# kalenforn/clip-based-cross-modal-hash

Measured on AMD Instinct MI355X. Metric: Hamming query x gallery pairs/sec (fused mAP@all pass, DCMHT COCO-shaped 64-bit), higher is better.
Workload: dtype u32; 1 GPU; configs[1] DCMHT COCO 64-bit retrieval: Q=5000 queries x R=117218 gallery items per GPU (x1 GPUs, contiguous shards), K=64 bits, C=80 classes, mAP@all; Q=5000, R_per_gpu=117218, K=64, C=80, parallelism=gallery-shard x1, query_blocks=1

## Files before the change

### clip-based-cross-modal-hash_amd/csrc/xmh_scan.hip

```cpp
#include "xmh_common.h"
#include <atomic>
#include <math.h>
#include <mutex>
#include <string.h>
#include <vector>
#include "xmh_scan_bits.h"
#include "xmh_scan_mfma.h"
#include "xmh_scan_kernels.h"

#include <stdlib.h>
#include <type_traits>
#include <unordered_set>

namespace {

constexpr int kSlotBudget64 = 9 * 1024;
constexpr int kSlotBudget32 = 5 * 1024;
constexpr int slots_for(int W, bool tern, int counter_bytes) {
    const int nbmax = (tern ? 64 : 32) * W + 1;
    const int budget = counter_bytes == 8 ? kSlotBudget64 : kSlotBudget32;
    const int cap = W > 8 ? 64 : 8;
    int S = 2;
    while (S < cap && nbmax * (64 / S) * counter_bytes > budget) S *= 2;
    return S;
}
inline int instance_words(int W) { return W <= 1 ? 1 : (W <= 2 ? 2 : (W <= 4 ? 4 : (W <= 8 ? 8 : (W <= 16 ? 16 : (W <= 32 ? 32 : 64))))); }
constexpr bool pair_cache_shape(int W, bool tern) { return !tern && (W == 1 || W == 2 || W == 4 || W == 8); }
template <int W, bool TERN>
constexpr bool kPairCacheShape = pair_cache_shape(W, TERN);
constexpr int cache_slots(int W) { return W <= 2 ? 4 : 8; }
static_assert(slots_for(2, false, 4) == 4 && slots_for(2, false, 8) == 4 && slots_for(4, false, 4) == 8 && slots_for(4, false, 8) == 8 &&
              slots_for(8, false, 4) == 8 && slots_for(8, false, 8) == 8, "33..256 bits: the cache geometry is the uncached kernels' own");
constexpr int waves_for(int W, bool tern) { return (W >= 32 && !tern) ? 8 : 1; }
inline size_t aos_ring_bytes(int W, int LW, bool tern) { return (size_t)64 * (((W * (tern ? 2 : 1) + LW) + 3) / 4 * 4) * 4; }

struct WsLayout {
    size_t chunk_hist, below, tot, dpre, cap, tick, gate, ap_part, pair_cache, total;
};

bool r2_selfcheck_ok();
inline bool mfma_env_on() {
    const char* e = getenv("XMH_SCAN_MFMA");
    return !(e && atoi(e) == 0);
}
struct Overrides {
    int mfma = -1;
    bool masked = false;
    bool describe = false;
};
enum class Family { kValu, kR2, kR2w, kBits, kTBits };
Family pass1_family(int K, bool ternary, const Overrides& ov) {
    if (ov.mfma == 0 || !mfma_env_on()) return Family::kValu;
    if (ternary) return K <= 256 ? Family::kTBits : Family::kValu;
    if (K > 128) return K <= 256 ? Family::kBits : Family::kValu;
    if (ov.mfma < 0 && !r2_selfcheck_ok()) return Family::kValu;
    return K <= 64 ? Family::kR2 : Family::kR2w;
}
inline int tbits_tiles(int K) { return K <= 64 ? 2 : (K <= 128 ? 4 : 8); }
inline int ap_r2_mode() {
    const char* e = getenv("XMH_SCAN_AP_R2");
    return e ? (atoi(e) != 0 ? 1 : 0) : 2;
}
constexpr int kAp2Waves = 4, kAp2Groups = 2;
constexpr int kMfmaWaves = 4;
static_assert(xmh::kScanBitsWaves == kMfmaWaves, "k_scan_hist_b takes the plan's query tiles of 64");
// ... 174 lines not shown
}

int packed_rank_bits(int K, int64_t R) {
    const char* e = getenv("XMH_SCAN_PACK32");
    if (e && e[0] == '0') return 0;
    if (!(K > 64 || (e && e[0] == 'a'))) return 0;
    const int64_t rank_max = R + 2;
    int rank_bits = 0;
    while ((1ll << rank_bits) < rank_max) ++rank_bits;
    return rank_bits > 24 ? 0 : rank_bits;
}

enum class Mode { kUnsharded, kBaseAll, kTotals, kAllToAll };
struct ScanCall {
    const uint32_t *qbits, *qzero, *qlab, *rbits, *rzero, *rlab;
    int64_t Q, R; int K, C;
    void* ws; size_t ws_bytes;
    bool tern;
};
struct Pass2 {
    Mode mode; int64_t k;
    double* ap_sum; int32_t* cap;
    double* map_out;
    const uint32_t *base_all = nullptr, *base_rel = nullptr, *nrel_total = nullptr;
    const uint32_t* hist_g = nullptr;
    int world = 0, rank = 0;
};
enum class Kern { kHistS, kHistR2, kHistR2w, kHistB, kApS, kApC, kApR2 };
enum Gate : unsigned {
    kBySize = 1,
    kByWrap = 2,
    kByWidth = 4,
};
struct Launch {
    Kern kern = Kern::kHistS;
    int W = 0, LW = 0;
    bool tern = false, cache = false;
    int S = 0, NW = 1;
    int nml = 0;
    int eb = 0; bool half = false;
    bool p32 = false, masked = false;
    unsigned gate = 0;
    bool stand_in = false;
};
struct ScanRoute {
    Launch p1;
    size_t cache_bytes = 0;
    int rank_bits = 0;
    Launch p2[3];
    int n2 = 0;
    bool tables32 = false;
};

std::mutex g_packed_mu;
std::unordered_set<const void*> g_packed_ws;
bool ws_packed(const void* ws) { std::lock_guard<std::mutex> lock(g_packed_mu); return g_packed_ws.count(ws) != 0; }
void ws_set_packed(const void* ws, bool on) {
    std::lock_guard<std::mutex> lock(g_packed_mu);
    if (on) g_packed_ws.insert(ws); else g_packed_ws.erase(ws);
}
bool counts_fit16(int K, int64_t R) {
    double peak = 1.0;
    for (int i = 1; i <= K / 2; ++i) peak *= (double)(K - K / 2 + i) / (double)i;
    peak = ldexp(peak, -K);
    return 2.0 * peak * (double)R <= 65535.0;
}
bool tables_packed(bool apc_alone, Mode mode, int K, int64_t R) { return apc_alone && mode == Mode::kUnsharded && counts_fit16(K, R); }

ScanRoute scan_route(const xmh_scan_plan& p, const ScanCall& c, Mode mode, const Overrides& ov, hipStream_t st) {
    ScanRoute r;
    const int K = c.K, C = c.C; const bool tern = c.tern; const int64_t R = c.R;
    const Family fam = pass1_family(K, tern, ov);
    const int W = ov.describe ? instance_words((K + 31) / 32) : (K + 31) / 32, LW = (C + 31) / 32;
    const bool lane_ok = ov.describe || (!ov.masked && lane_order_ok(st));
    r.cache_bytes = cache_for_workspace(p, K, tern, fam, c.ws_bytes);
    const bool cache = r.cache_bytes != 0;
    const bool mfma = fam != Family::kValu && LW <= 4 && lane_ok;
    Launch& h = r.p1;
    h.W = W; h.LW = LW; h.tern = tern; h.cache = cache; h.nml = LW <= 2 ? 1 : 2;
    if (!mfma) {
        h.cache = cache && pair_cache_shape(W, tern);
        h.S = h.cache ? cache_slots(W) : slots_for(W, tern, 4);
        h.NW = h.S == 64 ? waves_for(W, tern) : 1;
    } else if (fam == Family::kBits || fam == Family::kTBits) {
        h.kern = Kern::kHistB;
        h.S = fam == Family::kTBits ? tbits_tiles(K) : 4;
    } else {
        const R2Geom g = r2_geom(K);
        h.kern = fam == Family::kR2 ? Kern::kHistR2 : Kern::kHistR2w;
        h.NW = g.nw; h.S = g.nq;
    }
    const bool sharded = mode != Mode::kUnsharded;
    const bool masked = !lane_ok;
    const int rank_bits = sharded || masked ? 0 : packed_rank_bits(K, R);
    const bool fits_fb = sharded || R <= kFloatBitsMaxItems;
    const bool apc_on = ap_c_on();
    const bool byte128 = cache && mfma && fam == Family::kR2w;
    const bool tb = cache && mfma && fam == Family::kTBits;
    const bool apc = cache && apc_on && (byte128 || (K <= 64 && rank_bits == 0)) && !tern && !masked && (mode != Mode::kBaseAll || byte128) && fits_fb;
    const bool apr2 = !cache && mfma && fam == Family::kR2 && ap_r2_mode() != 0 && !masked && mode != Mode::kBaseAll && rank_bits == 0 && fits_fb;
    const bool apc16 = cache && apc_on && ((K > 128 && K <= 256 && !tern) || tb) && !masked && !sharded && R <= kFloatBitsMaxItems;
    const unsigned size_gate = sharded && (apc || apr2) ? kBySize : 0u;
    r.rank_bits = byte128 && apc ? 0 : rank_bits;
    auto add = [&](Kern kern, unsigned gate) -> Launch& { Launch& l = r.p2[r.n2++]; l.kern = kern; l.gate = gate; return l; };
    if (apc) {
        Launch& l = add(Kern::kApC, size_gate | (byte128 ? kByWrap : 0u));
        l.eb = 8; l.half = byte128; l.S = byte128 ? 8 : 4;
    }
    if (apr2) {
        Launch& l = add(Kern::kApR2, size_gate);
        l.W = W; l.LW = LW; l.nml = h.nml; l.NW = kAp2Waves; l.S = kAp2Groups;
    }
// ... 63 lines not shown
}

MfmaArgs r2_args(const ScanCall& c, const Launch& l, const xmh_scan_plan& p, int nqt) {
    MfmaArgs a{c.qbits, (int)c.Q, (int)c.R, c.K, l.W, (int)p.chunk, (int)p.nchunk, nqt, (int)p.nbuckets, (int)p.qpad};
    a.rbits = c.rbits; a.rlab = c.rlab; a.qlab = c.qlab; a.LW = l.LW;
    return a;
}

struct Geom { unsigned grid, block; size_t lds; int nqt, nrun; };
Geom launch_geom(const Launch& l, const xmh_scan_plan& p, int64_t Q) {
    const size_t nb = (size_t)p.nbuckets;
    const bool ap = l.kern == Kern::kApS || l.kern == Kern::kApC || l.kern == Kern::kApR2;
    Geom g{0, 64u * (unsigned)l.NW, 0, 0};
    if (l.kern == Kern::kHistS || l.kern == Kern::kApS) {
        g.lds = ((nb * (64 / l.S) * (ap && !l.p32 ? 2 : 1) + 3) & ~(size_t)3) * 4 * l.NW + (ap && l.cache ? 0 : aos_ring_bytes(l.W, l.LW, l.tern));
        g.nqt = (int)p.nqtile * l.S / l.NW;
    } else if (l.kern == Kern::kApC) {
        g.lds = nb * (64 / l.S) * 8; g.nqt = (int)p.nqtile * l.S;
    } else if (l.kern == Kern::kHistB) {
        g.nqt = (int)(p.qpad / (16 * kMfmaWaves));
    } else if (l.kern == Kern::kHistR2 || l.kern == Kern::kHistR2w) {
        g.lds = r2_lds_bytes(l.S, (int)nb); g.nqt = (int)(p.qpad / (l.NW * l.S * 16));
    } else {
        g.lds = (size_t)l.NW * l.S * nb * 16 * (ap ? 8 : 4); g.nqt = (int)(p.qpad / (l.NW * l.S * 16));
    }
    g.nrun = g.nqt;
    if (ap) {
        static const bool all_tiles = xmh_experiment_env("XMH_AP_TILES") && atoi(xmh_experiment_env("XMH_AP_TILES")) == 0;
        if (!all_tiles) g.nrun = (int)xmh::ceil_div(Q, p.qpad / g.nqt);
    }
    g.grid = xmh::scan_grid_blocks(g.nrun, (int)p.nchunk);
    return g;
}

template <typename KernT, typename... Args>
int start(const char* who, const Launch& l, const Geom& g, hipStream_t st, KernT kern, int S, int NW, bool cache, Args... args) {
    if (l.S != S || l.NW != NW || l.cache != cache)
        return xmh::fail(XMH_ENOTSUP, "%s: the route names an instance with S=%d NW=%d cache=%d, the one compiled for W=%d LW=%d has S=%d NW=%d cache=%d", who, l.S,
                         l.NW, (int)l.cache, l.W, l.LW, S, NW, (int)cache);
    if (const int rc = xmh::raise_dynamic_lds(reinterpret_cast<const void*>(kern), g.lds, who)) return rc;
    hipLaunchKernelGGL(kern, dim3(g.grid), dim3(g.block), g.lds, st, args...);
    return XMH_OK;
}

struct ScanCtx {
    const ScanCall& c;
    hipStream_t st;
    xmh_scan_plan p;
    ScanRoute r;
    WsLayout L;
    ScanArgs a;
    uint32_t kcap = 0xffffffffu;
    bool capped = false;
    template <typename T> T* at(size_t off) const { return reinterpret_cast<T*>(static_cast<char*>(c.ws) + off); }
    uint32_t* chunk_hist() const { return at<uint32_t>(L.chunk_hist); }
    uint32_t rel_scale() const { return r.p1.kern != Kern::kHistS ? kRelHi16 : 0u; }
    const uint2* below() const { return at<uint2>(L.below); }
    uint2* tot() const { return at<uint2>(L.tot); }
    uint2* dpre() const { return at<uint2>(L.dpre); }
    uint32_t* cap_ws() const { return at<uint32_t>(L.cap); }
    float* ap_part() const { return at<float>(L.ap_part); }
    ScanArgs args(const Geom& g, bool cached) const { ScanArgs as = a; as.nqt = g.nqt; as.nrun = g.nrun; as.pair_cache = cached ? pair_cache() : nullptr; return as; }
    uint32_t* gate(int word = 0) const { return at<uint32_t>(L.gate) + word; }
    const uint32_t* gate_if(const Launch& l, unsigned g, int word) const { return (l.gate & g) ? gate(word) : nullptr; }
    uint4* pair_cache() const { return r.cache_bytes ? at<uint4>(L.pair_cache) : nullptr; }
};

int plan_call(const char* who, ScanCtx& x, const Overrides& ov) {
    if (const int rc = make_plan(x.c.Q, x.c.R, x.c.K, x.c.tern, &x.p, ov)) return rc;
    return check_common(who, x.c, x.p);
}
void route_call(ScanCtx& x, Mode mode, const Overrides& ov) {
    x.r = scan_route(x.p, x.c, mode, ov, x.st);
    x.a = make_args(x.c, x.p);
    x.L = ws_layout(x.p, x.r.cache_bytes);
}

int valu_hist(const ScanCtx& x) {
    const Launch& h = x.r.p1;
    const Geom g = launch_geom(h, x.p, x.c.Q);
    const ScanArgs as = x.args(g, h.cache);
    auto go = [&](auto kern, int S, int NW, bool cache) {
        xmh::ProfScope prof("scan_hist", x.st);
        return start("xmh_hamming_hist", h, g, x.st, kern, S, NW, cache, as, x.chunk_hist());
    };
    auto launch = [&](auto tern_c) {
        constexpr bool T = decltype(tern_c)::value;
        return dispatch_shape<T>(h.W, h.LW, [&](auto w, auto l) {
            constexpr int WW = decltype(w)::value, LL = decltype(l)::value;
            if constexpr (kPairCacheShape<WW, T>) {
                if (h.cache) return go(k_scan_hist_s<WW, LL, T, cache_slots(WW), 1, true>, cache_slots(WW), 1, true);
            }
            constexpr int S = slots_for(WW, T, 4);
            constexpr int NW = S == 64 ? waves_for(WW, T) : 1;
            return go(k_scan_hist_s<WW, LL, T, S, NW, false>, S, NW, false);
        });
    };
    return h.tern ? launch(std::true_type{}) : launch(std::false_type{});
}

int mfma_hist(const ScanCtx& x) {
    const Launch& h = x.r.p1;
    const xmh_scan_plan& p = x.p;
    const Geom g = launch_geom(h, p, x.c.Q);
    uint32_t* chunk_hist = x.chunk_hist();
    uint4* cache = x.pair_cache();
    if (h.kern == Kern::kHistB) {
        xmh::ScanBitsArgs a{x.c.rbits, x.c.rlab, x.c.qbits, x.c.qlab, (int)x.c.Q, (int)x.c.R, x.c.K, h.W, h.LW, (int)p.chunk, (int)p.nchunk, g.nqt,
                            (int)p.nbuckets, (int)p.qpad};
        a.rzero = x.c.rzero; a.qzero = x.c.qzero;
        return xmh::launch_scan_hist_bits(a, h.S, chunk_hist, cache, x.st);
    }
    hipLaunchKernelGGL(k_scan_touch, dim3(xmh::scan_grid_blocks(kTouchPerChunk, (int)p.nchunk)), dim3(256), 0, x.st, x.c.rbits, x.c.rlab, x.c.R, h.W, h.LW,
                       p.chunk, (int)p.nchunk, x.at<uint32_t>(x.L.tick), (int)((x.L.gate + 256 - x.L.tick) / 4));
    XMH_LAUNCH_CHECK("xmh_hamming_hist control words");
    const MfmaArgs a = r2_args(x.c, h, p, g.nqt);
    xmh::ProfScope prof("scan_hist", x.st);
    auto go = [&](auto kern, int NW, int NQ, bool cached, auto... wrap_word) { return start("xmh_hamming_hist", h, g, x.st, kern, NQ, NW, cached, a, chunk_hist, cache, wrap_word...); };
    if (h.kern == Kern::kHistR2w) {
        uint32_t* ovf = x.gate(kGateWrapped);
        return h.nml == 1 ? (h.cache ? go(k_scan_hist_r2w<1, 4, 2, true>, 4, 2, true, ovf) : go(k_scan_hist_r2w<1, 4, 2, false>, 4, 2, false, ovf))
                          : (h.cache ? go(k_scan_hist_r2w<2, 4, 2, true>, 4, 2, true, ovf) : go(k_scan_hist_r2w<2, 4, 2, false>, 4, 2, false, ovf));
    }
    return h.nml == 1 ? (h.cache ? go(k_scan_hist_r2<1, 4, 4, true>, 4, 4, true) : go(k_scan_hist_r2<1, 4, 4, false>, 4, 4, false))
                      : (h.cache ? go(k_scan_hist_r2<2, 4, 4, true>, 4, 4, true) : go(k_scan_hist_r2<2, 4, 4, false>, 4, 4, false));
}

int hamming_hist_impl(const ScanCall& c, uint32_t* hist_all, uint32_t* hist_rel, xmh_stream_t stream, const Overrides& ov, bool pass2_sharded = false) {
    ScanCtx x{c, xmh::as_stream(stream)};
    if (const int rc = plan_call("xmh_hamming_hist", x, ov)) return rc;
    route_call(x, Mode::kUnsharded, ov);
    const xmh_scan_plan& p = x.p;
    const Kern kern = x.r.p1.kern;
    const bool packed = x.r.tables32 && !pass2_sharded;
    if (kern == Kern::kHistS || kern == Kern::kHistB) XMH_HIP(hipMemsetAsync(x.at<char>(x.L.tick), 0, x.L.gate + 256 - x.L.tick, x.st));
    if (const int rc = kern == Kern::kHistS ? valu_hist(x) : mfma_hist(x)) return rc;
    XMH_LAUNCH_CHECK("xmh_hamming_hist");
    hipLaunchKernelGGL(k_scan_below, dim3((unsigned)p.nqtile, (unsigned)xmh::ceil_div(p.nbuckets, 4)), dim3(256), 0, x.st, x.chunk_hist(), (int)p.qpad,
                       (int)p.nbuckets, (int)p.nchunk, x.rel_scale(), x.at<uint2>(x.L.below), x.tot(), x.at<uint32_t>(x.L.tick), (int)c.Q, x.dpre(),
                       x.cap_ws(), x.gate(), hist_all, hist_rel, packed, x.gate(kGateWide));
    XMH_LAUNCH_CHECK("xmh_hamming_hist below");
    ws_set_packed(c.ws, packed);
    return XMH_OK;
}

}

extern "C" int xmh_scan_plan_make(int64_t Q, int64_t R, int K, int ternary, xmh_scan_plan* plan_host) {
    if (!plan_host) return xmh::fail(XMH_EINVAL, "xmh_scan_plan_make: null plan");
    return make_plan(Q, R, K, ternary, plan_host);
}

extern "C" size_t xmh_scan_pair_cache_bytes(int64_t Q, int64_t R, int K, int ternary) {
    xmh_scan_plan p;
    if (make_plan(Q, R, K, ternary, &p)) return 0;
    return pair_cache_bytes(p, K, ternary != 0, pass1_family(K, ternary != 0, {}));
}

extern "C" size_t xmh_scan_pair_cache_offset(int64_t Q, int64_t R, int K, int ternary) {
    xmh_scan_plan p;
    if (make_plan(Q, R, K, ternary, &p)) return (size_t)-1;
    return ws_layout(p, 0).pair_cache;
}

extern "C" size_t xmh_scan_ws_bytes_nocache(int64_t Q, int64_t R, int K, int ternary) {
    xmh_scan_plan p;
    if (make_plan(Q, R, K, ternary, &p)) return 0;
    return ws_layout(p, 0).total;
}

extern "C" int xmh_scan_describe(int64_t Q, int64_t R, int K, int C, int ternary, char* out, size_t out_bytes) {
    if (!out || out_bytes < 64) return xmh::fail(XMH_EINVAL, "xmh_scan_describe: buffer too small");
    xmh_scan_plan p;
    if (const int rc = make_plan(Q, R, K, ternary, &p)) return rc;
    Overrides ov;
    ov.describe = true;
    const ScanCall c{nullptr, nullptr, nullptr, nullptr, nullptr, nullptr, Q, R, K, C, nullptr, (size_t)p.ws_bytes, ternary != 0};
    const ScanRoute r = scan_route(p, c, Mode::kUnsharded, ov, nullptr);
    char p1[160], p2[200] = "", one[120];
    if (const int rc = describe_launch(r.p1, p1, sizeof(p1))) return rc;
    for (const bool p32 : {true, false})
        for (int i = 0; i < r.n2; ++i) {
            if (r.p2[i].stand_in || r.p2[i].p32 != p32) continue;
            if (const int rc = describe_launch(r.p2[i], one, sizeof(one))) return rc;
            const size_t at = strlen(p2);
            snprintf(p2 + at, sizeof(p2) - at, "%s%s", at ? "|" : "", one);
        }
    if ((size_t)snprintf(out, out_bytes, "pass1=%s;pass2=%s", p1, p2) >= out_bytes) return xmh::fail(XMH_EINVAL, "xmh_scan_describe: buffer too small");
    return XMH_OK;
}

extern "C" size_t xmh_scan_gate_offset(int64_t Q, int64_t R, int K, int ternary) {
    xmh_scan_plan p;
    if (make_plan(Q, R, K, ternary, &p)) return (size_t)-1;
    return ws_layout(p, 0).gate;
// ... 2 lines not shown
extern "C" int xmh_scan_tables_packed(int64_t Q, int64_t R, int K, int C, int ternary, int mode) {
    if (mode < 0 || mode > 3) return xmh::fail(XMH_EINVAL, "xmh_scan_tables_packed: mode=%d", mode);
    xmh_scan_plan p;
    if (const int rc = make_plan(Q, R, K, ternary, &p)) return rc;
    Overrides ov;
    ov.describe = true;
    const ScanCall c{nullptr, nullptr, nullptr, nullptr, nullptr, nullptr, Q, R, K, C, nullptr, (size_t)p.ws_bytes, ternary != 0};
    static const Mode modes[4] = {Mode::kUnsharded, Mode::kBaseAll, Mode::kTotals, Mode::kAllToAll};
    return scan_route(p, c, modes[mode], ov, nullptr).tables32 ? 1 : 0;
}

extern "C" int xmh_hamming_hist(const uint32_t* qbits, const uint32_t* qzero, const uint32_t* qlab,
                                const uint32_t* rbits, const uint32_t* rzero, const uint32_t* rlab, int64_t Q, int64_t R,
                                int K, int C, void* ws, size_t ws_bytes, uint32_t* hist_all, uint32_t* hist_rel,
                                xmh_stream_t stream) {
    XMH_RANGE("xmh_hamming_hist (pass 1)");
    const ScanCall c{qbits, qzero, qlab, rbits, rzero, rlab, Q, R, K, C, ws, ws_bytes, qzero != nullptr};
    return hamming_hist_impl(c, hist_all, hist_rel, stream, {}, hist_all != nullptr || hist_rel != nullptr);
}

extern "C" int xmh_hamming_hist_for(const uint32_t* qbits, const uint32_t* qzero, const uint32_t* qlab,
                                    const uint32_t* rbits, const uint32_t* rzero, const uint32_t* rlab, int64_t Q, int64_t R,
                                    int K, int C, void* ws, size_t ws_bytes, uint32_t* hist_all, uint32_t* hist_rel, int pass2_sharded,
                                    xmh_stream_t stream) {
    XMH_RANGE("xmh_hamming_hist (pass 1)");
    const ScanCall c{qbits, qzero, qlab, rbits, rzero, rlab, Q, R, K, C, ws, ws_bytes, qzero != nullptr};
    return hamming_hist_impl(c, hist_all, hist_rel, stream, {}, pass2_sharded != 0);
}

namespace {
int ap_offsets(const ScanCtx& x, const Pass2& o) {
    const xmh_scan_plan& p = x.p;
    if (o.mode == Mode::kUnsharded) return XMH_OK;
    if (o.mode == Mode::kAllToAll)
        hipLaunchKernelGGL(k_shard_scatter_offsets, dim3((unsigned)xmh::ceil_div(p.qpad, 256), (unsigned)p.nbuckets + 1), dim3(256), 0, x.st,
                           reinterpret_cast<const uint2*>(o.hist_g), (int)p.nbuckets, (int)(p.qpad / o.world), (int)x.c.Q, (int)p.qpad, o.k, x.dpre(), x.cap_ws(),
                           o.cap, x.gate(2));
    else if (o.mode == Mode::kTotals)
        hipLaunchKernelGGL(k_shard_offsets_dpre, dim3((unsigned)p.nqtile), dim3(256), 0, x.st, reinterpret_cast<const uint2*>(o.hist_g), o.world, o.rank,
                           (int)x.c.Q, (int)p.qpad, (int)p.nbuckets, o.k, x.dpre(), x.cap_ws(), o.cap, x.gate(2));
    else
        hipLaunchKernelGGL(k_scan_dpre, dim3((unsigned)p.nqtile), dim3(256), 0, x.st, (const uint2*)x.tot(), (int)x.c.Q, (int)p.qpad, (int)p.nbuckets, o.base_all,
                           o.base_rel, o.nrel_total, o.k, x.dpre(), x.cap_ws(), o.cap, (uint32_t*)nullptr, (uint32_t*)nullptr, (uint32_t*)nullptr, x.gate(2));
    XMH_LAUNCH_CHECK(o.mode == Mode::kAllToAll ? "xmh_hamming_map_sharded_offsets scatter" : (o.mode == Mode::kTotals ? "xmh_hamming_map_sharded offsets" : "xmh_hamming_ap dpre"));
    return XMH_OK;
}

int ap_launch_c(const ScanCtx& x, const Launch& l) {
    const Geom g = launch_geom(l, x.p, x.c.Q);
    const ScanArgs as = x.args(g, true);
    const uint32_t* wide = x.r.tables32 ? x.gate(kGateWide) : nullptr;
    xmh::ProfScope prof("scan_ap", x.st);
    auto go = [&](auto kc, int S) {
        return start("xmh_hamming_ap", l, g, x.st, kc, S, 1, l.cache, as, x.below(), (const uint2*)x.dpre(), (const uint32_t*)x.cap_ws(), x.ap_part(),
                     x.gate_if(l, kBySize, 2), x.kcap, x.gate_if(l, kByWrap, kGateWrapped), x.gate_if(l, kByWidth, 0), l.gate & kByWidth ? x.r.rank_bits : 0, wide,
                     (const uint32_t*)x.chunk_hist(), x.rel_scale());
    };
    if (l.eb == 16) return x.capped ? go(k_scan_ap_c<true, 16>, 8) : go(k_scan_ap_c<false, 16>, 8);
    if (l.half) return x.capped ? go(k_scan_ap_c<true, 8, true>, 8) : go(k_scan_ap_c<false, 8, true>, 8);
    return x.capped ? go(k_scan_ap_c<true, 8>, 4) : go(k_scan_ap_c<false, 8>, 4);
}

int ap_launch_r2(const ScanCtx& x, const Launch& l) {
    const Geom g = launch_geom(l, x.p, x.c.Q);
    const MfmaArgs ma = r2_args(x.c, l, x.p, g.nrun);
    xmh::ProfScope prof("scan_ap", x.st);
    auto go = [&](auto kern) {
        return start("xmh_hamming_ap", l, g, x.st, kern, kAp2Groups, kAp2Waves, l.cache, ma, x.below(), (const uint2*)x.dpre(), (const uint32_t*)x.cap_ws(), x.ap_part(),
                     x.gate_if(l, kBySize, 2), x.kcap);
    };
    return l.nml == 1 ? (x.capped ? go(k_scan_ap_r2<1, kAp2Waves, kAp2Groups, true>) : go(k_scan_ap_r2<1, kAp2Waves, kAp2Groups, false>))
                      : (x.capped ? go(k_scan_ap_r2<2, kAp2Waves, kAp2Groups, true>) : go(k_scan_ap_r2<2, kAp2Waves, kAp2Groups, false>));
}

int ap_launch_s(const ScanCtx& x, const Launch& l) {
    const Geom g = launch_geom(l, x.p, x.c.Q);
    const ScanArgs as = x.args(g, l.cache);
    auto go = [&](auto kern, int S, int NW, bool cache, const uint32_t* run_if) {
        xmh::ProfScope prof(l.p32 ? "scan_ap32" : "scan_ap", x.st);
        return start("xmh_hamming_ap", l, g, x.st, kern, S, NW, cache, as, x.below(), (const uint2*)x.dpre(), (const uint32_t*)x.cap_ws(), x.ap_part(),
                     (const uint32_t*)x.gate(), x.r.rank_bits, x.kcap, x.gate_if(l, kBySize, 2), run_if);
    };
    auto by_shape = [&](auto tern_c, auto cap_c, auto p32_c, auto masked_c) {
        constexpr bool T = decltype(tern_c)::value, CP = decltype(cap_c)::value, P32 = decltype(p32_c)::value, MK = decltype(masked_c)::value;
        return dispatch_shape<T>(l.W, l.LW, [&](auto w, auto lw) {
            constexpr int WW = decltype(w)::value, LL = decltype(lw)::value;
            if constexpr (P32 && MK) return xmh::fail(XMH_ENOTSUP, "xmh_hamming_ap: the masked fallback runs 64-bit counters only");
            else {
                if constexpr (kPairCacheShape<WW, T> && !MK) {
                    if (l.cache)
                        return go(k_scan_ap_s<WW, 1, T, CP, cache_slots(WW), P32, MK, 1, true>, cache_slots(WW), 1, true, nullptr);
                }
                (void)CP;
                constexpr int S = slots_for(WW, T, P32 ? 4 : 8);
                constexpr int NW = S == 64 ? waves_for(WW, T) : 1;
                return go(k_scan_ap_s<WW, LL, T, true, S, P32, MK, NW, false>, S, NW, false, x.gate_if(l, kByWrap, kGateWrapped));
            }
        });
    };
    using T1 = std::true_type; using T0 = std::false_type;
    auto by_mask = [&](auto t, auto c, auto w) { return l.masked ? by_shape(t, c, w, T1{}) : by_shape(t, c, w, T0{}); };
    auto by_width = [&](auto t, auto c) { return l.p32 ? by_mask(t, c, T1{}) : by_mask(t, c, T0{}); };
    auto by_cap = [&](auto t) { return x.capped ? by_width(t, T1{}) : by_width(t, T0{}); };
    return l.tern ? by_cap(T1{}) : by_cap(T0{});
}

int ap_reduce(const ScanCtx& x, const Pass2& o) {
    const int64_t Q = x.c.Q;
    const unsigned nred = (unsigned)xmh::ceil_div(Q, 64);
// ... 15 lines not shown

static std::atomic<int> g_verify{0};
constexpr int XMH_EVERIFY_CODE = -74;

int hamming_ap_impl(const ScanCall& c, const Pass2& o, xmh_stream_t stream, const Overrides& ov);

int verify_against_masked(const ScanCall& c, const Pass2& o, xmh_stream_t stream) {
    hipStream_t st = xmh::as_stream(stream);
    const int64_t Q = c.Q;
    std::vector<double> a1((size_t)Q), a0((size_t)Q);
    std::vector<int32_t> c1((size_t)Q), c0((size_t)Q);
    XMH_HIP(hipMemcpyAsync(a1.data(), o.ap_sum, (size_t)Q * 8, hipMemcpyDeviceToHost, st));
    XMH_HIP(hipMemcpyAsync(c1.data(), o.cap, (size_t)Q * 4, hipMemcpyDeviceToHost, st));
    XMH_HIP(hipStreamSynchronize(st));
    Overrides ov;
    ov.mfma = 0;
    ov.masked = true;
    xmh_scan_plan p;
    if (const int rc = make_plan(Q, c.R, c.K, c.tern, &p, ov)) return rc;
    const size_t small = ws_layout(p, 0).total;
    DevBuf ws2, ap2, cap2;
    if (!ws2.alloc(small) || !ap2.alloc((size_t)Q * 8) || !cap2.alloc((size_t)Q * 4))
        return xmh::fail(XMH_ENOMEM, "xmh_scan_verify: no room for the second evaluation (%zu bytes)", small);
    ScanCall again = c; again.ws = ws2.p; again.ws_bytes = small;
    const Pass2 o2{Mode::kUnsharded, o.k, ap2.as<double>(), cap2.as<int32_t>(), nullptr};
    if (const int rc = hamming_hist_impl(again, nullptr, nullptr, stream, ov)) return rc;
    if (const int rc = hamming_ap_impl(again, o2, stream, ov)) return rc;
    XMH_HIP(hipMemcpyAsync(a0.data(), ap2.p, (size_t)Q * 8, hipMemcpyDeviceToHost, st));
    XMH_HIP(hipMemcpyAsync(c0.data(), cap2.p, (size_t)Q * 4, hipMemcpyDeviceToHost, st));
    XMH_HIP(hipStreamSynchronize(st));
    if (const char* fe = getenv("XMH_SCAN_VERIFY_FAULT")) {
        const int64_t at = atoll(fe) % Q;
        a1[(size_t)at] *= 1.0 + 1e-3;
    }
    int64_t bad = -1, nbad = 0;
    for (int64_t i = 0; i < Q; ++i) {
        const bool same = c1[(size_t)i] == c0[(size_t)i] && fabs(a1[(size_t)i] - a0[(size_t)i]) <= 4e-6 * fabs(a0[(size_t)i]) + 1e-9;
        if (!same) { if (bad < 0) bad = i; ++nbad; }
    }
    if (nbad)
        return xmh::fail(XMH_EVERIFY_CODE, "xmh_scan_verify: %lld of %lld queries differ between the lane-order kernels and the masked re-derivation "
                         "(first: query %lld, AP sum %.9g vs %.9g, divisor %d vs %d)", (long long)nbad, (long long)Q, (long long)bad, a1[(size_t)bad], a0[(size_t)bad],
                         c1[(size_t)bad], c0[(size_t)bad]);
    return XMH_OK;
}

int hamming_ap_impl(const ScanCall& c, const Pass2& o, xmh_stream_t stream, const Overrides& ov) {
    ScanCtx x{c, xmh::as_stream(stream)};
    if (const int rc = plan_call("xmh_hamming_ap", x, ov)) return rc;
    if (!o.ap_sum || !o.cap) return xmh::fail(XMH_EINVAL, "xmh_hamming_ap: null output");
    const int ext = (o.base_all != nullptr) + (o.base_rel != nullptr) + (o.nrel_total != nullptr);
    if (ext != 0 && ext != 3) return xmh::fail(XMH_EINVAL, "xmh_hamming_ap: base_all, base_rel and nrel_total go together");
    route_call(x, o.mode, ov);
    const bool have_packed = ws_packed(c.ws);
    if (x.r.tables32 && !have_packed) x.r.tables32 = false;
    x.kcap = o.k > 0 && o.k < (int64_t)0xffffffffll ? (uint32_t)o.k : 0xffffffffu;
    x.capped = o.k > 0;
    if (!x.r.tables32 && have_packed) {
        const xmh_scan_plan& p = x.p;
        hipLaunchKernelGGL(k_scan_below, dim3((unsigned)p.nqtile, (unsigned)xmh::ceil_div(p.nbuckets, 4)), dim3(256), 0, x.st, x.chunk_hist(), (int)p.qpad,
                           (int)p.nbuckets, (int)p.nchunk, x.rel_scale(), x.at<uint2>(x.L.below), x.tot(), (uint32_t*)nullptr, (int)x.c.Q, (uint2*)nullptr,
                           (uint32_t*)nullptr, (uint32_t*)nullptr, (uint32_t*)nullptr, (uint32_t*)nullptr, false, (uint32_t*)nullptr);
        XMH_LAUNCH_CHECK("xmh_hamming_ap below");
        ws_set_packed(c.ws, false);
    }
    if (const int rc = ap_offsets(x, o)) return rc;
    for (int i = 0; i < x.r.n2; ++i) {
        const Launch& l = x.r.p2[i];
        if (const int rc = l.kern == Kern::kApC ? ap_launch_c(x, l) : (l.kern == Kern::kApR2 ? ap_launch_r2(x, l) : ap_launch_s(x, l))) return rc;
        XMH_LAUNCH_CHECK("xmh_hamming_ap");
    }
    if (const int rc = ap_reduce(x, o)) return rc;
    if (g_verify.load(std::memory_order_relaxed) && !ov.masked && o.mode == Mode::kUnsharded) return verify_against_masked(c, o, stream);
    return XMH_OK;
}

bool selfcheck_eval(const ScanCall& c, int force, std::vector<uint32_t>& hist, std::vector<double>& ap, std::vector<int32_t>& cap) {
    Overrides ov;
    ov.mfma = force;
    const int64_t Q = c.Q;
    xmh_scan_plan p;
    if (make_plan(Q, c.R, c.K, 0, &p, ov) != XMH_OK) return false;
    const size_t nb = (size_t)p.nbuckets;
    DevBuf ws, dh, dap, dcap;
    if (!ws.alloc(p.ws_bytes) || !dh.alloc(2 * Q * nb * 4) || !dap.alloc(Q * 8) || !dcap.alloc(Q * 4)) return false;
    ScanCall run = c; run.ws = ws.p; run.ws_bytes = p.ws_bytes;
    const Pass2 o{Mode::kUnsharded, 0, dap.as<double>(), dcap.as<int32_t>(), nullptr};
    uint32_t* h = dh.as<uint32_t>();
    if (hamming_hist_impl(run, h, h + Q * nb, nullptr, ov) != XMH_OK) return false;
    if (hamming_ap_impl(run, o, nullptr, ov) != XMH_OK) return false;
    hist.resize(2 * Q * nb); ap.resize(Q); cap.resize(Q);
    if (hipDeviceSynchronize() != hipSuccess) return false;
    return hipMemcpy(hist.data(), dh.p, hist.size() * 4, hipMemcpyDeviceToHost) == hipSuccess && hipMemcpy(ap.data(), dap.p, Q * 8, hipMemcpyDeviceToHost) == hipSuccess &&
           hipMemcpy(cap.data(), dcap.p, Q * 4, hipMemcpyDeviceToHost) == hipSuccess;
}

bool r2_selfcheck_ok() {
    static int state[64];
    static std::mutex mu;
    int dev = 0;
    if (hipGetDevice(&dev) != hipSuccess || dev < 0 || dev >= 64) return true;
    const char* e = getenv("XMH_SCAN_M2_SELFCHECK");
    if (e && atoi(e) == 0) return true;
    std::lock_guard<std::mutex> lock(mu);
    if (state[dev]) return state[dev] == 1;
    state[dev] = 1;
    const int64_t Q = 272, R = 9000;
    bool same = true, ran = true;
    {
        const void* const r2_kernels[] = {reinterpret_cast<const void*>(k_scan_hist_r2<1, 4, 4, true>), reinterpret_cast<const void*>(k_scan_hist_r2<1, 4, 4, false>),
                                          reinterpret_cast<const void*>(k_scan_hist_r2<2, 4, 4, true>), reinterpret_cast<const void*>(k_scan_hist_r2<2, 4, 4, false>),
                                          reinterpret_cast<const void*>(k_scan_hist_r2w<1, 4, 2, true>), reinterpret_cast<const void*>(k_scan_hist_r2w<1, 4, 2, false>),
                                          reinterpret_cast<const void*>(k_scan_hist_r2w<2, 4, 2, true>), reinterpret_cast<const void*>(k_scan_hist_r2w<2, 4, 2, false>)};
        for (const void* k : r2_kernels) {
            hipFuncAttributes fa;
            if (hipFuncGetAttributes(&fa, k) != hipSuccess) ran = false;
            else if (fa.sharedSizeBytes != 0) same = false;
// ... 160 lines not shown
```

### clip-based-cross-modal-hash_amd/csrc/xmh_scan_kernels.h

```cpp
#pragma once
#include "xmh_scan_mfma.h"

namespace {
template <int W, int LW, bool TERN>
struct QueryRegs {
    uint32_t b[W];
    uint32_t z[TERN ? W : 1];
    uint32_t l[LW];
    __device__ __forceinline__ void load(const ScanArgs& a, int q) {
        const bool ok = q < a.Q;
#pragma unroll
        for (int w = 0; w < W; ++w) b[w] = ok ? a.qbits[(int64_t)q * W + w] : 0u;
        if (TERN) {
#pragma unroll
            for (int w = 0; w < W; ++w) z[w] = ok ? a.qzero[(int64_t)q * W + w] : 0xffffffffu;
        }
#pragma unroll
        for (int w = 0; w < LW; ++w) l[w] = ok ? a.qlab[(int64_t)q * LW + w] : 0u;
    }
};

template <int W, int LW, bool TERN>
struct Rec {
    uint32_t b[W];
// ... 7 lines not shown
        int acc = 0;
#pragma unroll
        for (int w = 0; w < W; ++w) acc += __popc(qr.b[w] ^ r.b[w]);
        d = acc;
    } else {
        int live_n = 0, diff_n = 0;
#pragma unroll
        for (int w = 0; w < W; ++w) {
            const uint32_t live = ~(qr.z[w] | r.z[w]);
            live_n += __popc(live);
            diff_n += __popc((qr.b[w] ^ r.b[w]) & live);
        }
        d = K - live_n + 2 * diff_n;
    }
    uint32_t hit = qr.l[0] & r.l[0];
#pragma unroll
    for (int w = 1; w < LW; ++w) asm("v_and_or_b32 %0, %1, %2, %0" : "+v"(hit) : "v"(qr.l[w]), "v"(r.l[w]));
    asm("v_min_u32 %0, %1, 1" : "=v"(hit01) : "v"(hit));
}

constexpr int kGateWrapped = 3;
constexpr int kGateWide = 4;
__global__ __launch_bounds__(256) void k_scan_below(const uint32_t* __restrict__ chunk_hist, int qpad, int nb, int nchunk, uint32_t rel_scale,
                                                    uint2* __restrict__ below, uint2* __restrict__ tot, uint32_t* __restrict__ tickets, int Q,
                                                    uint2* __restrict__ dpre, uint32_t* __restrict__ nrel_ws, uint32_t* __restrict__ nrel_max,
                                                    uint32_t* __restrict__ hist_all, uint32_t* __restrict__ hist_rel, bool packed,
                                                    uint32_t* __restrict__ wide) {
    __shared__ uint2 part[4][64];
    __shared__ int last;
    const int lane = threadIdx.x & 63, wq = threadIdx.x >> 6;
    const int d = blockIdx.y * 4 + wq;
    const int q = blockIdx.x * 64 + lane;
    const bool hi16 = rel_scale == kRelHi16;
    if (d < nb && packed) {
        const int64_t cell = (int64_t)d * qpad + q, step = (int64_t)nb * qpad;
        const uint32_t* __restrict__ src = chunk_hist + cell;
        uint32_t* __restrict__ dst = reinterpret_cast<uint32_t*>(below) + cell;
        uint32_t ra = 0, rr = 0;
        for (int c0 = 0; c0 < nchunk; c0 += 16) {
            uint32_t h[16];
#pragma unroll
            for (int j = 0; j < 16; ++j, src += step) h[j] = c0 + j < nchunk ? *src : 0u;
#pragma unroll
            for (int j = 0; j < 16; ++j, dst += step) {
                if (c0 + j < nchunk) {
                    *dst = (ra << 16) | rr;
                    const uint2 n = chunk_counts(h[j], rel_scale);
                    ra += n.x;
                    rr += n.y;
                }
            }
        }
        if (ra > 0xffffu && q < Q) *wide = 1u;
        __hip_atomic_store(reinterpret_cast<unsigned long long*>(tot + (int64_t)d * qpad + q), (unsigned long long)ra | ((unsigned long long)rr << 32),
                           __ATOMIC_RELAXED, __HIP_MEMORY_SCOPE_AGENT);
    } else if (d < nb) {
        uint32_t ra = 0, rr = 0;
        int c = 0;
        for (; c + 4 <= nchunk; c += 4) {
            uint32_t h[4];
#pragma unroll
            for (int j = 0; j < 4; ++j) h[j] = chunk_hist[((int64_t)(c + j) * nb + d) * qpad + q];
#pragma unroll
            for (int j = 0; j < 4; ++j) {
                below[((int64_t)(c + j) * nb + d) * qpad + q] = make_uint2(ra, rr);
                const uint32_t rel = hi16 ? h[j] & 0xffffu : (rel_scale ? h[j] / rel_scale : h[j] >> 16);
                ra += hi16 ? h[j] >> 16 : (rel_scale ? h[j] - rel * rel_scale : h[j] & 0xffffu);
                rr += rel;
            }
        }
        for (; c < nchunk; ++c) {
            const uint32_t h = chunk_hist[((int64_t)c * nb + d) * qpad + q];
            below[((int64_t)c * nb + d) * qpad + q] = make_uint2(ra, rr);
            const uint32_t rel = hi16 ? h & 0xffffu : (rel_scale ? h / rel_scale : h >> 16);
            ra += hi16 ? h >> 16 : (rel_scale ? h - rel * rel_scale : h & 0xffffu);
            rr += rel;
        }
        __hip_atomic_store(reinterpret_cast<unsigned long long*>(tot + (int64_t)d * qpad + q), (unsigned long long)ra | ((unsigned long long)rr << 32),
                           __ATOMIC_RELAXED, __HIP_MEMORY_SCOPE_AGENT);
    }
    if (!tickets) return;
    asm volatile("s_waitcnt vmcnt(0)" ::: "memory");
    __syncthreads();
    if (threadIdx.x == 0) {
        const uint32_t t = __hip_atomic_fetch_add(tickets + blockIdx.x, 1u, __ATOMIC_RELAXED, __HIP_MEMORY_SCOPE_AGENT);
        last = t == gridDim.y - 1;
    }
    __syncthreads();
    if (!last) return;
    auto tot_at = [&](int dd) {
        const unsigned long long v = __hip_atomic_load(reinterpret_cast<const unsigned long long*>(tot + (int64_t)dd * qpad + q), __ATOMIC_RELAXED,
                                                       __HIP_MEMORY_SCOPE_AGENT);
        return make_uint2((uint32_t)v, (uint32_t)(v >> 32));
    };
    const int nbq = (nb + 3) / 4;
    const int d0 = wq * nbq, d1 = (d0 + nbq < nb) ? d0 + nbq : nb;
    uint32_t sa = 0, sr = 0;
    for (int dd = d0; dd < d1; dd += 8) {
        uint2 t[8];
#pragma unroll
        for (int j = 0; j < 8; ++j) t[j] = dd + j < d1 ? tot_at(dd + j) : make_uint2(0u, 0u);
#pragma unroll
        for (int j = 0; j < 8; ++j) { sa += t[j].x; sr += t[j].y; }
    }
    part[wq][lane] = make_uint2(sa, sr);
    __syncthreads();
    uint32_t ra = 0, rr = 0, tr = 0;
#pragma unroll
// ... 841 lines not shown
```

### clip-based-cross-modal-hash_amd/csrc/xmh_scan_mfma.h

```cpp
#pragma once
#include "xmh_common.h"
#include "xmh_scan_map.h"
#include <type_traits>
#include <utility>

namespace {

constexpr int kMaxChunk = 32768;
constexpr uint32_t kF23 = 0x4B000000u;
constexpr int64_t kFloatBitsMaxItems = (1ll << 23) - 3;
constexpr int kMinChunk = 256;
constexpr uint32_t kRelHi16 = 0xffffffffu;
__device__ __forceinline__ uint2 chunk_counts(uint32_t h, uint32_t rel_scale) {
    if (rel_scale == kRelHi16) return make_uint2(h >> 16, h & 0xffffu);
    if (rel_scale == 0u) return make_uint2(h & 0xffffu, h >> 16);
    return make_uint2(h % rel_scale, h / rel_scale);
}

struct ScanArgs {
    const uint32_t* qbits;
    const uint32_t* qzero;
    const uint32_t* qlab;
    const uint32_t* rbits;
    const uint32_t* rzero;
// ... 573 lines not shown
            uint32_t i0, i1, i2, i3;
            consume(i0, i1, i2, i3, A[3]);
            if (CACHE) pack(cw[NQ - 1][3], addr_p, i0, i1, i2, i3);
        }
#ifdef XMH_ABL_NOSTORE
        if (CACHE && a.Q < 0) {
#else
        if (CACHE) {
#endif
#pragma unroll
            for (int h = 0; h < NQ; ++h) {
                uint4* dst = crow[h] + (int64_t)i * 64;
                __builtin_nontemporal_store(cw[h][0], &dst->x);
                __builtin_nontemporal_store(cw[h][1], &dst->y);
                __builtin_nontemporal_store(cw[h][2], &dst->z);
                __builtin_nontemporal_store(cw[h][3], &dst->w);
            }
        }
#pragma unroll
        for (int g = 0; g < 4; ++g)
#pragma unroll
            for (int m = 0; m < NMI; ++m) wcur[g][m] = wnxt[g][m];
    }
    const int npad = nbat * 64 - (int)(hi - lo);
    asm volatile("s_waitcnt lgkmcnt(0)" ::: "memory");
    if (npad > 0 && slot == 0) {
#pragma unroll
        for (int h = 0; h < NQ; ++h) {
            if (!valid[h]) continue;
            const int64_t q = (int64_t)(t16 + h) * 16 + ql;
            int dpad = 0;
            for (int w = 0; w < a.W; ++w) dpad += __popc(a.qbits[q * a.W + w]);
            lds[r2_cell(wave, h, dpad, ql)] -= (uint32_t)npad << 16;
        }
    }
#pragma unroll
    for (int h = 0; h < NQ; ++h) {
        uint32_t* __restrict__ out = chunk_hist + ((int64_t)chunk_id * a.nb) * a.qpad + (t16 + h) * 16;
        for (int e = lane; e < ncell; e += 64) out[(int64_t)(e >> 4) * a.qpad + (e & 15)] = lds[r2_cell(wave, h, e >> 4, e & 15)];
    }
    if (CACHE && dmax >= 65536u) *ovf = 1u;
}
#undef XMH_W_FUSED
#undef XMH_W_MFMA_F4
#undef XMH_W_MFMA
#undef XMH_W_MIN
#undef XMH_W_ADD

template <bool CAPPED, int EB, bool HALF = false>
__global__ __launch_bounds__(64) void k_scan_ap_c(ScanArgs a, const uint2* __restrict__ below, const uint2* __restrict__ dpre,
                                                  const uint32_t* __restrict__ cap_ws, float* __restrict__ ap_part,
                                                  const uint32_t* __restrict__ items_total, uint32_t kcap, const uint32_t* __restrict__ skip_if = nullptr,
                                                  const uint32_t* __restrict__ nrel_max = nullptr, int rank_bits = 0, const uint32_t* __restrict__ wide = nullptr,
                                                  const uint32_t* __restrict__ chunk_hist = nullptr, uint32_t rel_scale = 0) {
    static_assert(!HALF || EB == 8, "the 8 x 8 geometry on one-byte entries");
    constexpr int QW = HALF ? 8 : 128 / EB, LOG_QW = QW == 16 ? 4 : 3, S = 64 / QW, EPW = HALF ? 2 : 32 / EB;
    extern __shared__ __attribute__((aligned(16))) uint32_t lds[];
    int chunk_id, qtile;
    if (!map_block(a, chunk_id, qtile)) return;
    if (items_total && (int64_t)*items_total > kFloatBitsMaxItems) return;
    if (skip_if && *skip_if != 0u) return;
    if (nrel_max && rank_bits > 0 && (uint64_t)(*nrel_max) + 2 < (1ull << (32 - rank_bits))) return;
    const int lane = threadIdx.x & 63;
    const int ql = lane & (QW - 1), slot = lane >> LOG_QW;
    const int q0 = qtile * QW, q = q0 + ql;
    const int ncell = a.nb * QW;
    unsigned long long* cnt = reinterpret_cast<unsigned long long*>(lds);
    {
        const uint2* __restrict__ pb = below + ((int64_t)chunk_id * a.nb) * a.qpad + q0;
        const uint2* __restrict__ pd = dpre + q0;
        auto pack = [](uint2 x, uint2 y) {
            return (unsigned long long)(kF23 + x.x + y.x + 1u) | ((unsigned long long)(kF23 + (0x7fffffu - (x.y + y.y + 1u))) << 32);
        };
        int e = lane;
        if (wide == nullptr) {
            for (; e + 7 * 64 < ncell; e += 8 * 64) {
                uint2 x[8], y[8];
#pragma unroll
                for (int j = 0; j < 8; ++j) {
                    const int ee = e + j * 64;
                    const int64_t at = (int64_t)(ee >> LOG_QW) * a.qpad + (ee & (QW - 1));
                    x[j] = pb[at];
                    y[j] = pd[at];
                }
#pragma unroll
                for (int j = 0; j < 8; ++j) cnt[e + j * 64] = pack(x[j], y[j]);
            }
            for (; e < ncell; e += 64) {
                const int64_t at = (int64_t)(e >> LOG_QW) * a.qpad + (e & (QW - 1));
                cnt[e] = pack(pb[at], pd[at]);
            }
        } else if (*wide == 0u) {
            const uint32_t* __restrict__ pw = reinterpret_cast<const uint32_t*>(below) + ((int64_t)chunk_id * a.nb) * a.qpad + q0;
            auto unpack = [](uint32_t w) { return make_uint2(w >> 16, w & 0xffffu); };
            for (; e + 7 * 64 < ncell; e += 8 * 64) {
                uint32_t w[8];
                uint2 y[8];
#pragma unroll
                for (int j = 0; j < 8; ++j) {
                    const int ee = e + j * 64;
                    const int64_t at = (int64_t)(ee >> LOG_QW) * a.qpad + (ee & (QW - 1));
                    w[j] = pw[at];
                    y[j] = pd[at];
                }
#pragma unroll
                for (int j = 0; j < 8; ++j) cnt[e + j * 64] = pack(unpack(w[j]), y[j]);
            }
            for (; e < ncell; e += 64) {
                const int64_t at = (int64_t)(e >> LOG_QW) * a.qpad + (e & (QW - 1));
                cnt[e] = pack(unpack(pw[at]), pd[at]);
            }
        } else {
            const uint32_t* __restrict__ ph = chunk_hist + q0;
            for (; e < ncell; e += 64) {
                const int64_t at = (int64_t)(e >> LOG_QW) * a.qpad + (e & (QW - 1));
                uint2 x = make_uint2(0u, 0u);
#pragma unroll 4
                for (int c = 0; c < chunk_id; ++c) {
                    const uint2 n = chunk_counts(ph[((int64_t)c * a.nb) * a.qpad + at], rel_scale);
                    x.x += n.x;
                    x.y += n.y;
                }
                cnt[e] = pack(x, pd[at]);
            }
        }
    }
    asm volatile("" : "+s"(ap_part));
    const uint32_t cntbase = (uint32_t)(uintptr_t)(__attribute__((address_space(3))) uint32_t*)lds + ql * 8;
    const float capf = CAPPED ? (float)min(cap_ws[q], kcap) : 0.0f;
    const int64_t lo = (int64_t)chunk_id * a.chunk;
    const int64_t hi = (lo + a.chunk < a.R) ? lo + a.chunk : a.R;
    float acc = 0.0f;
    auto credit = [&](unsigned long long old, uint32_t m) {
        const float rank = __uint_as_float((uint32_t)old) - 8388608.0f;
        const float ord = 16777215.0f - __uint_as_float((uint32_t)(old >> 32));
        if (CAPPED) m = ord <= capf ? m : 0u;
#ifdef XMH_ABL_AP_NORCP
        acc = fmaf(ord, __uint_as_float(__float_as_uint(rank) & m), acc);
#else
        acc = fmaf(ord, __uint_as_float(__float_as_uint(__builtin_amdgcn_rcpf(rank)) & m), acc);
#endif
    };
    const uint32_t hoff = HALF ? 8u * (uint32_t)(slot >> 2) : 0u;
    const uint32_t hb0 = hoff, hb1 = hoff + 16u, hd0 = hoff + 1u, hd1 = hoff + 17u;
    auto issue1 = [&](uint32_t w, int j, unsigned long long& old, uint32_t& m) {
        uint32_t d;
        if (HALF) {
            m = (uint32_t)__builtin_amdgcn_sbfe((int)w, j ? hb1 : hb0, 1);
            d = __builtin_amdgcn_ubfe(w, j ? hd1 : hd0, EB - 1);
        } else if (EB == 16) {
            m = (uint32_t)__builtin_amdgcn_sbfe((int)w, j, 1);
            d = __builtin_amdgcn_ubfe(w, j + 1, 11);
        } else {
            m = (uint32_t)__builtin_amdgcn_sbfe((int)w, EB * j, 1);
            d = __builtin_amdgcn_ubfe(w, EB * j + 1, EB - 1);
        }
        uint32_t addr;
        if (QW == 16) asm("v_lshl_add_u32 %0, %1, 7, %2" : "=v"(addr) : "v"(d), "v"(cntbase));
        else asm("v_lshl_add_u32 %0, %1, 6, %2" : "=v"(addr) : "v"(d), "v"(cntbase));
        const unsigned long long inc = 1ull | ((unsigned long long)m << 32);
#ifdef XMH_ABL_AP_NOATOMIC
        old = ((unsigned long long)addr << 3) | inc;
        asm volatile("" : "+v"(old));
#else
        asm volatile("ds_add_rtn_u64 %0, %1, %2" : "=v"(old) : "v"(addr), "v"(inc) : "memory");
#endif
    };
    unsigned long long oldA[8], oldB[8];
    uint32_t mA[8], mB[8];
    constexpr bool kFourBatchIterations = true;
    auto issue = [&](unsigned long long (&old)[8], uint32_t (&m)[8], uint32_t wa, uint32_t wb, uint32_t wc, uint32_t wd) {
        if constexpr (EB == 16) {
            const uint32_t sx = __builtin_amdgcn_alignbit(wb, wa, 24), sy = __builtin_amdgcn_alignbit(wc, wb, 28);
#pragma unroll
            for (int u = 0; u < 8; ++u) issue1(XMH_CACHE12_WORD(u, wa, wb, wc, sx, sy), XMH_CACHE12_BIT(u), old[u], m[u]);
        } else {
#pragma unroll
            for (int u = 0; u < 8; ++u) {
                const int wi = u / EPW;
                issue1(wi == 0 ? wa : (wi == 1 ? wb : (wi == 2 ? wc : wd)), u % EPW, old[u], m[u]);
            }
        }
// ... 408 lines not shown
```

Measured before the change: 1841 billion pairs/s.

## Fuse the distance-prefix tail of the below scan into the AP kernel

When packed 16-bit tables are used and the caller does not need the histogram outputs, the below-scan kernel now skips its ticketed tail, which computed per-distance prefix sums and per-query relevant totals. The AP kernel instead reads the per-distance totals, builds the exclusive prefix per slot with wave shuffles, and writes the relevant count itself. The goal is to remove the serialized ticket/tail work and one global round trip between kernels. The cost is redundant prefix computation in every AP block, plus added state tracking so a fallback path can rebuild the tail when it is needed.

```diff
diff --git a/clip-based-cross-modal-hash_amd/csrc/xmh_scan.hip b/clip-based-cross-modal-hash_amd/csrc/xmh_scan.hip
--- a/clip-based-cross-modal-hash_amd/csrc/xmh_scan.hip
+++ b/clip-based-cross-modal-hash_amd/csrc/xmh_scan.hip
@@ -10,7 +10,7 @@
 
 #include <stdlib.h>
 #include <type_traits>
-#include <unordered_set>
+#include <unordered_map>
 
 namespace {
 
@@ -291,12 +291,17 @@
     bool tables32 = false;
 };
 
+enum class Tables { k64, kPacked, kPackedNoTail };
 std::mutex g_packed_mu;
-std::unordered_set<const void*> g_packed_ws;
-bool ws_packed(const void* ws) { std::lock_guard<std::mutex> lock(g_packed_mu); return g_packed_ws.count(ws) != 0; }
-void ws_set_packed(const void* ws, bool on) {
+std::unordered_map<const void*, Tables> g_packed_ws;
+Tables ws_tables(const void* ws) {
     std::lock_guard<std::mutex> lock(g_packed_mu);
-    if (on) g_packed_ws.insert(ws); else g_packed_ws.erase(ws);
+    const auto it = g_packed_ws.find(ws);
+    return it == g_packed_ws.end() ? Tables::k64 : it->second;
+}
+void ws_set_tables(const void* ws, Tables t) {
+    std::lock_guard<std::mutex> lock(g_packed_mu);
+    if (t == Tables::k64) g_packed_ws.erase(ws); else g_packed_ws[ws] = t;
 }
 bool counts_fit16(int K, int64_t R) {
     double peak = 1.0;
@@ -466,6 +471,7 @@
     ScanArgs a;
     uint32_t kcap = 0xffffffffu;
     bool capped = false;
+    bool no_tail = false;
     template <typename T> T* at(size_t off) const { return reinterpret_cast<T*>(static_cast<char*>(c.ws) + off); }
     uint32_t* chunk_hist() const { return at<uint32_t>(L.chunk_hist); }
     uint32_t rel_scale() const { return r.p1.kern != Kern::kHistS ? kRelHi16 : 0u; }
@@ -547,14 +553,15 @@
     const xmh_scan_plan& p = x.p;
     const Kern kern = x.r.p1.kern;
     const bool packed = x.r.tables32 && !pass2_sharded;
+    const bool no_tail = packed && !hist_all && !hist_rel;
     if (kern == Kern::kHistS || kern == Kern::kHistB) XMH_HIP(hipMemsetAsync(x.at<char>(x.L.tick), 0, x.L.gate + 256 - x.L.tick, x.st));
     if (const int rc = kern == Kern::kHistS ? valu_hist(x) : mfma_hist(x)) return rc;
     XMH_LAUNCH_CHECK("xmh_hamming_hist");
     hipLaunchKernelGGL(k_scan_below, dim3((unsigned)p.nqtile, (unsigned)xmh::ceil_div(p.nbuckets, 4)), dim3(256), 0, x.st, x.chunk_hist(), (int)p.qpad,
-                       (int)p.nbuckets, (int)p.nchunk, x.rel_scale(), x.at<uint2>(x.L.below), x.tot(), x.at<uint32_t>(x.L.tick), (int)c.Q, x.dpre(),
-                       x.cap_ws(), x.gate(), hist_all, hist_rel, packed, x.gate(kGateWide));
+                       (int)p.nbuckets, (int)p.nchunk, x.rel_scale(), x.at<uint2>(x.L.below), x.tot(), no_tail ? (uint32_t*)nullptr : x.at<uint32_t>(x.L.tick), (int)c.Q,
+                       x.dpre(), x.cap_ws(), x.gate(), hist_all, hist_rel, packed, x.gate(kGateWide));
     XMH_LAUNCH_CHECK("xmh_hamming_hist below");
-    ws_set_packed(c.ws, packed);
+    ws_set_tables(c.ws, no_tail ? Tables::kPackedNoTail : (packed ? Tables::kPacked : Tables::k64));
     return XMH_OK;
 }
 
@@ -663,9 +670,9 @@
     const uint32_t* wide = x.r.tables32 ? x.gate(kGateWide) : nullptr;
     xmh::ProfScope prof("scan_ap", x.st);
     auto go = [&](auto kc, int S) {
-        return start("xmh_hamming_ap", l, g, x.st, kc, S, 1, l.cache, as, x.below(), (const uint2*)x.dpre(), (const uint32_t*)x.cap_ws(), x.ap_part(),
+        return start("xmh_hamming_ap", l, g, x.st, kc, S, 1, l.cache, as, x.below(), (const uint2*)(x.no_tail ? x.tot() : x.dpre()), (const uint32_t*)x.cap_ws(), x.ap_part(),
                      x.gate_if(l, kBySize, 2), x.kcap, x.gate_if(l, kByWrap, kGateWrapped), x.gate_if(l, kByWidth, 0), l.gate & kByWidth ? x.r.rank_bits : 0, wide,
-                     (const uint32_t*)x.chunk_hist(), x.rel_scale());
+                     (const uint32_t*)x.chunk_hist(), x.rel_scale(), x.no_tail ? x.cap_ws() : (uint32_t*)nullptr);
     };
     if (l.eb == 16) return x.capped ? go(k_scan_ap_c<true, 16>, 8) : go(k_scan_ap_c<false, 16>, 8);
     if (l.half) return x.capped ? go(k_scan_ap_c<true, 8, true>, 8) : go(k_scan_ap_c<false, 8, true>, 8);
@@ -787,17 +794,22 @@
     const int ext = (o.base_all != nullptr) + (o.base_rel != nullptr) + (o.nrel_total != nullptr);
     if (ext != 0 && ext != 3) return xmh::fail(XMH_EINVAL, "xmh_hamming_ap: base_all, base_rel and nrel_total go together");
     route_call(x, o.mode, ov);
-    const bool have_packed = ws_packed(c.ws);
+    const Tables have = ws_tables(c.ws);
+    const bool have_packed = have != Tables::k64;
     if (x.r.tables32 && !have_packed) x.r.tables32 = false;
+    x.no_tail = x.r.tables32 && have == Tables::kPackedNoTail;
     x.kcap = o.k > 0 && o.k < (int64_t)0xffffffffll ? (uint32_t)o.k : 0xffffffffu;
     x.capped = o.k > 0;
     if (!x.r.tables32 && have_packed) {
         const xmh_scan_plan& p = x.p;
+        const bool tail = have == Tables::kPackedNoTail;
+        if (tail) XMH_HIP(hipMemsetAsync(x.at<char>(x.L.tick), 0, x.L.gate - x.L.tick, x.st));
         hipLaunchKernelGGL(k_scan_below, dim3((unsigned)p.nqtile, (unsigned)xmh::ceil_div(p.nbuckets, 4)), dim3(256), 0, x.st, x.chunk_hist(), (int)p.qpad,
-                           (int)p.nbuckets, (int)p.nchunk, x.rel_scale(), x.at<uint2>(x.L.below), x.tot(), (uint32_t*)nullptr, (int)x.c.Q, (uint2*)nullptr,
-                           (uint32_t*)nullptr, (uint32_t*)nullptr, (uint32_t*)nullptr, (uint32_t*)nullptr, false, (uint32_t*)nullptr);
+                           (int)p.nbuckets, (int)p.nchunk, x.rel_scale(), x.at<uint2>(x.L.below), x.tot(), tail ? x.at<uint32_t>(x.L.tick) : (uint32_t*)nullptr, (int)x.c.Q,
+                           tail ? x.dpre() : (uint2*)nullptr, tail ? x.cap_ws() : (uint32_t*)nullptr, tail ? x.gate() : (uint32_t*)nullptr, (uint32_t*)nullptr,
+                           (uint32_t*)nullptr, false, (uint32_t*)nullptr);
         XMH_LAUNCH_CHECK("xmh_hamming_ap below");
-        ws_set_packed(c.ws, false);
+        ws_set_tables(c.ws, Tables::k64);
     }
     if (const int rc = ap_offsets(x, o)) return rc;
     for (int i = 0; i < x.r.n2; ++i) {
diff --git a/clip-based-cross-modal-hash_amd/csrc/xmh_scan_kernels.h b/clip-based-cross-modal-hash_amd/csrc/xmh_scan_kernels.h
--- a/clip-based-cross-modal-hash_amd/csrc/xmh_scan_kernels.h
+++ b/clip-based-cross-modal-hash_amd/csrc/xmh_scan_kernels.h
@@ -83,8 +83,10 @@
             }
         }
         if (ra > 0xffffu && q < Q) *wide = 1u;
-        __hip_atomic_store(reinterpret_cast<unsigned long long*>(tot + (int64_t)d * qpad + q), (unsigned long long)ra | ((unsigned long long)rr << 32),
-                           __ATOMIC_RELAXED, __HIP_MEMORY_SCOPE_AGENT);
+        if (!tickets) tot[(int64_t)d * qpad + q] = make_uint2(ra, rr);
+        else
+            __hip_atomic_store(reinterpret_cast<unsigned long long*>(tot + (int64_t)d * qpad + q), (unsigned long long)ra | ((unsigned long long)rr << 32),
+                               __ATOMIC_RELAXED, __HIP_MEMORY_SCOPE_AGENT);
     } else if (d < nb) {
         uint32_t ra = 0, rr = 0;
         int c = 0;
diff --git a/clip-based-cross-modal-hash_amd/csrc/xmh_scan_mfma.h b/clip-based-cross-modal-hash_amd/csrc/xmh_scan_mfma.h
--- a/clip-based-cross-modal-hash_amd/csrc/xmh_scan_mfma.h
+++ b/clip-based-cross-modal-hash_amd/csrc/xmh_scan_mfma.h
@@ -649,7 +649,8 @@
                                                   const uint32_t* __restrict__ cap_ws, float* __restrict__ ap_part,
                                                   const uint32_t* __restrict__ items_total, uint32_t kcap, const uint32_t* __restrict__ skip_if = nullptr,
                                                   const uint32_t* __restrict__ nrel_max = nullptr, int rank_bits = 0, const uint32_t* __restrict__ wide = nullptr,
-                                                  const uint32_t* __restrict__ chunk_hist = nullptr, uint32_t rel_scale = 0) {
+                                                  const uint32_t* __restrict__ chunk_hist = nullptr, uint32_t rel_scale = 0,
+                                                  uint32_t* __restrict__ nrel_out = nullptr) {
     static_assert(!HALF || EB == 8, "the 8 x 8 geometry on one-byte entries");
     constexpr int QW = HALF ? 8 : 128 / EB, LOG_QW = QW == 16 ? 4 : 3, S = 64 / QW, EPW = HALF ? 2 : 32 / EB;
     extern __shared__ __attribute__((aligned(16))) uint32_t lds[];
@@ -663,6 +664,7 @@
     const int q0 = qtile * QW, q = q0 + ql;
     const int ncell = a.nb * QW;
     unsigned long long* cnt = reinterpret_cast<unsigned long long*>(lds);
+    uint32_t nrel_q = 0u;
     {
         const uint2* __restrict__ pb = below + ((int64_t)chunk_id * a.nb) * a.qpad + q0;
         const uint2* __restrict__ pd = dpre + q0;
@@ -670,7 +672,62 @@
             return (unsigned long long)(kF23 + x.x + y.x + 1u) | ((unsigned long long)(kF23 + (0x7fffffu - (x.y + y.y + 1u))) << 32);
         };
         int e = lane;
-        if (wide == nullptr) {
+        if (nrel_out != nullptr) {
+            const int rpp = (a.nb + S - 1) / S;
+            const int d0 = slot * rpp < a.nb ? slot * rpp : a.nb, d1 = d0 + rpp < a.nb ? d0 + rpp : a.nb;
+            const uint2* __restrict__ pt = dpre + q;
+            uint32_t sa = 0u, sr = 0u;
+            for (int d = d0; d < d1; d += 8) {
+                uint2 t[8];
+#pragma unroll
+                for (int j = 0; j < 8; ++j) t[j] = d + j < d1 ? pt[(int64_t)(d + j) * a.qpad] : make_uint2(0u, 0u);
+#pragma unroll
+                for (int j = 0; j < 8; ++j) { sa += t[j].x; sr += t[j].y; }
+            }
+            uint32_t ra = 0u, rr = 0u;
+#pragma unroll
+            for (int j = 0; j < S; ++j) {
+                const uint32_t pa = (uint32_t)__shfl((int)sa, j * QW + ql), pr = (uint32_t)__shfl((int)sr, j * QW + ql);
+                if (j < slot) { ra += pa; rr += pr; }
+                nrel_q += pr;
+            }
+            if (chunk_id == 0 && slot == 0 && q < a.Q) nrel_out[q] = nrel_q;
+            if (*wide == 0u) {
+                const uint32_t* __restrict__ pw = reinterpret_cast<const uint32_t*>(below) + ((int64_t)chunk_id * a.nb) * a.qpad + q;
+                for (int d = d0; d < d1; d += 8) {
+                    uint2 t[8];
+                    uint32_t w[8];
+#pragma unroll
+                    for (int j = 0; j < 8; ++j) {
+                        const int64_t at = (int64_t)(d + j) * a.qpad;
+                        t[j] = d + j < d1 ? pt[at] : make_uint2(0u, 0u);
+                        w[j] = d + j < d1 ? pw[at] : 0u;
+                    }
+#pragma unroll
+                    for (int j = 0; j < 8; ++j) {
+                        if (d + j < d1) cnt[(d + j) * QW + ql] = pack(make_uint2(w[j] >> 16, w[j] & 0xffffu), make_uint2(ra, rr));
+                        ra += t[j].x;
+                        rr += t[j].y;
+                    }
+                }
+            } else {
+                const uint32_t* __restrict__ ph = chunk_hist + q;
+                for (int d = d0; d < d1; ++d) {
+                    const int64_t at = (int64_t)d * a.qpad;
+                    uint2 x = make_uint2(0u, 0u);
+#pragma unroll 4
+                    for (int c = 0; c < chunk_id; ++c) {
+                        const uint2 n = chunk_counts(ph[((int64_t)c * a.nb) * a.qpad + at], rel_scale);
+                        x.x += n.x;
+                        x.y += n.y;
+                    }
+                    cnt[d * QW + ql] = pack(x, make_uint2(ra, rr));
+                    const uint2 t = pt[at];
+                    ra += t.x;
+                    rr += t.y;
+                }
+            }
+        } else if (wide == nullptr) {
             for (; e + 7 * 64 < ncell; e += 8 * 64) {
                 uint2 x[8], y[8];
 #pragma unroll
@@ -724,7 +781,7 @@
     }
     asm volatile("" : "+s"(ap_part));
     const uint32_t cntbase = (uint32_t)(uintptr_t)(__attribute__((address_space(3))) uint32_t*)lds + ql * 8;
-    const float capf = CAPPED ? (float)min(cap_ws[q], kcap) : 0.0f;
+    const float capf = CAPPED ? (float)min(nrel_out ? nrel_q : cap_ws[q], kcap) : 0.0f;
     const int64_t lo = (int64_t)chunk_id * a.chunk;
     const int64_t hi = (lo + a.chunk < a.R) ? lo + a.chunk : a.R;
     float acc = 0.0f;
```

After: 1870 billion pairs/s, median of 6. 1.5% higher.
